# UWQuickstep/quickstep

Hardware: AMD Instinct MI355X
Metric: probe+aggregate rows/s at TPC-H SF100 (Q1,Q3) (higher is better)
Workload: dtype i32 keys / f64 sums

## Files before the change

### quickstep_amd/csrc/join.hip

```cpp

#include "common.hpp"
#include "join_dense.hpp"
#include "join_lds.hpp"
#include "scan.hpp"

#include <atomic>
#include <cstdlib>
#include <vector>
#include <mutex>
#include <shared_mutex>
#include <type_traits>

namespace qsx {

constexpr int kJBlock = 256;
constexpr uint64_t kEmpty64 = ~0ull;
constexpr uint32_t kEmptyTid = 0xFFFFFFFFu;

struct alignas(16) LongEntry {
  int64_t key;
  uint32_t tid;
  uint32_t pad;
};

// ... 559 lines not shown
      __syncthreads();
      const unsigned long long base = s_base;
      for (int i = threadIdx.x; i < staged; i += kJBlock) {
        const unsigned long long o = base + i;
        if (o < sink.capacity) {
          __builtin_nontemporal_store(s_probe[i], &out_probe[o]);
          __builtin_nontemporal_store(s_build[i], &out_build[o]);
        }
      }
      __syncthreads();
    }
  }
  if (MODE != 0) {
    local_count = wave_reduce_add(local_count);
    if (lane_id() == 0 && local_count != 0 && out_count != nullptr) atomicAdd(out_count, local_count);
  }
}

}
#include "join_lds_bucket.hpp"
namespace qsx {

struct KeyPackArgs {
  const void *cols[QSX_MAX_KEYS];
  int is_long[QSX_MAX_KEYS];
  int shift[QSX_MAX_KEYS];
  int ncols;
  int exact;
};

__device__ __forceinline__ uint64_t combine_hashes(uint64_t first, uint64_t second) {
  const uint64_t kMul = 0x9ddfea08eb382d69ull;
  uint64_t a = (first ^ second) * kMul;
  a ^= (a >> 47);
  uint64_t b = (second ^ a) * kMul;
  b ^= (b >> 47);
  b *= kMul;
  return b;
}

__global__ __launch_bounds__(kJBlock) void key_pack_kernel(KeyPackArgs a, int64_t n, int64_t *__restrict__ out) {
  for (int64_t i = static_cast<int64_t>(blockIdx.x) * kJBlock + threadIdx.x; i < n;
       i += static_cast<int64_t>(gridDim.x) * kJBlock) {
    uint64_t acc = 0;
    for (int k = 0; k < a.ncols; ++k) {
      const uint64_t v = a.is_long[k] ? static_cast<uint64_t>(static_cast<const int64_t *>(a.cols[k])[i])
                                      : static_cast<uint64_t>(static_cast<const uint32_t *>(a.cols[k])[i]);
      if (a.exact) acc |= v << a.shift[k];
      else acc = k == 0 ? v : combine_hashes(acc, v);
    }
    out[i] = static_cast<int64_t>(acc);
  }
}

__global__ __launch_bounds__(kJBlock) void key_pack_char_kernel(const unsigned char *__restrict__ col, int width, int64_t n,
                                                               int64_t *__restrict__ out) {
  for (int64_t i = static_cast<int64_t>(blockIdx.x) * kJBlock + threadIdx.x; i < n; i += static_cast<int64_t>(gridDim.x) * kJBlock) {
    uint64_t key = 0;
    bool ended = false;
    for (int b = 0; b < width; ++b) {
      const unsigned char c = col[i * width + b];
      ended = ended || c == 0;
      key |= static_cast<uint64_t>(ended ? 0 : c) << (8 * b);
    }
    out[i] = static_cast<int64_t>(key);
  }
}

__global__ __launch_bounds__(kJBlock) void key_pack_runs_kernel(KeyPackArgs a, const long long *__restrict__ runs, long long cols_offset,
                                                               int64_t *__restrict__ out, int coded) {
  constexpr int kTileRows = 512;
  const int lane = lane_id();
  const int num_tiles = static_cast<int>(runs[2]);
  for (int tile = __builtin_amdgcn_readfirstlane(static_cast<int>(blockIdx.x * (kJBlock / kWave) + (threadIdx.x >> 6))); tile < num_tiles;
       tile += static_cast<int>(gridDim.x) * (kJBlock / kWave)) {
    const RunTile at = run_locate(runs, tile);
    const long long n = run_rows(runs, at.block);
    const long long out_first = run_base(runs, at.block);
    const long long *cols = runs + cols_offset + static_cast<long long>(at.block) * a.ncols;
    const long long total_entries = runs[0] * a.ncols;
    const long long *widths = cols + total_entries, *dicts = widths + total_entries;
    for (int r = lane; r < kTileRows; r += kWave) {
      const long long i = static_cast<long long>(at.tile_in_block) * kTileRows + r;
      if (i >= n) break;
      uint64_t acc = 0;
      for (int k = 0; k < a.ncols; ++k) {
        const void *col = as_global(reinterpret_cast<const void *>(cols[k]));
        const int code_width = coded != 0 ? static_cast<int>(widths[k]) : 0;
        uint64_t v;
        if (code_width == 0) {
          v = a.is_long[k] ? static_cast<uint64_t>(static_cast<const int64_t *>(col)[i]) : static_cast<uint64_t>(static_cast<const uint32_t *>(col)[i]);
        } else {
          const uint32_t code = code_width == 1 ? static_cast<const uint8_t *>(col)[i]
                                                : (code_width == 2 ? static_cast<const uint16_t *>(col)[i] : static_cast<const uint32_t *>(col)[i]);
          const void *dict = as_global(reinterpret_cast<const void *>(dicts[k]));
          if (dict == nullptr) v = code;
          else v = a.is_long[k] ? static_cast<uint64_t>(static_cast<const int64_t *>(dict)[code]) : static_cast<uint64_t>(static_cast<const uint32_t *>(dict)[code]);
        }
        if (a.exact) acc |= v << a.shift[k];
        else acc = k == 0 ? v : combine_hashes(acc, v);
      }
      out[out_first + i] = static_cast<int64_t>(acc);
    }
  }
}

}

using namespace qsx;

struct qsx_join_table {
  int key_type = QSX_INT;
  uint64_t capacity = 0;
  void *slots = nullptr;
  unsigned long long *entries_dev = nullptr;
  int64_t reserved = 0;
  std::atomic<int64_t> max_tid{-1};
  std::shared_mutex mutex;


  std::mutex seal_mutex;
  std::atomic<int> seal_state{0};
  std::atomic<bool> scanned{false};
  std::mutex marks_mutex;
  std::vector<std::pair<hipStream_t, hipEvent_t>> marks;
  unsigned long long *control_host = nullptr;
  hipEvent_t seal_event = nullptr;
  hipStream_t seal_stream = nullptr;
  void *compact = nullptr;
  uint64_t compact_capacity = 0;
  CompactView compact_view() const {
    return CompactView{static_cast<const uint32_t *>(compact), static_cast<const unsigned char *>(compact) + compact_capacity * 4};
  }
  std::mutex cover_mutex;
  std::vector<long long> cover_sig;
  void *cover = nullptr;
  size_t cover_bytes = 0;
  int cover_entry_bytes = 0;
  int cover_state = 0;
  hipEvent_t cover_event = nullptr;
  hipStream_t cover_stream = nullptr;
  qsx_join_table *shadow = nullptr;

  bool dense = false;
  int64_t min_key = 0;
  int stride_shift = 0;
  uint64_t range = 0;
  uint32_t *head = nullptr;
  unsigned char *head3 = nullptr;
  hipEvent_t pack_event = nullptr;
  hipStream_t pack_stream = nullptr;
  uint2 *ov = nullptr;
  unsigned int ov_capacity = 0;
  DenseTableView dense_view() const {
    DenseTableView v;
    v.head = head;
    v.head3 = seal_state.load(std::memory_order_acquire) == 2 ? head3 : nullptr;
    v.ov = ov;
    v.min_key = min_key;
    v.stride_shift = stride_shift;
    v.range = range;
    v.ov_count = reinterpret_cast<unsigned int *>(entries_dev + 2);
    v.ov_capacity = ov_capacity;
    v.error = reinterpret_cast<int *>(entries_dev + 3);
    return v;
  }

  size_t entry_bytes() const { return key_type == QSX_INT ? 8 : 16; }
  size_t table_bytes() const { return capacity * entry_bytes() + capacity; }
  static size_t alloc_bytes(size_t entry, uint64_t cap) { return cap * entry + cap + cap / kBucketSlots * sizeof(unsigned int); }
  uint64_t room() const { return capacity / 5 * 4; }
  TableView view() const {
    TableView v{};
    v.slots = slots;
    v.dup_flag = reinterpret_cast<unsigned int *>(entries_dev + 2);
    v.fp = static_cast<unsigned char *>(slots) + capacity * entry_bytes();
    v.buckets = capacity / kBucketSlots;
    v.fill = reinterpret_cast<unsigned int *>(v.fp + capacity);
    return v;
  }
};
static void drop_cover(qsx_join_table *t);

constexpr size_t kControlBytes = static_cast<size_t>(kControlReplicas) * kControlStride * sizeof(unsigned long long);
static int reset_control_words(unsigned long long *control, hipStream_t stream) {
  QSX_HIP_TRY(hipMemsetAsync(control, 0, kControlBytes, stream));
  return QSX_OK;
}
static bool fold_control_words(const unsigned long long *copies, unsigned long long *v) {
  unsigned long long entries = 0, lo_inv = 0, hi = 0;
  for (int r = 0; r < kControlReplicas; ++r) {
    const unsigned long long *c = copies + static_cast<size_t>(r) * kControlStride;
    entries += c[0];
    lo_inv = c[4] > lo_inv ? c[4] : lo_inv;
    hi = c[5] > hi ? c[5] : hi;
  }
  v[0] = entries;
  v[1] = 0;
  v[2] = copies[2];
  v[3] = copies[3];
  v[4] = ~lo_inv;
  v[5] = hi;
  return !(lo_inv == 0 && hi == 0);
}
static int copy_control_words(const unsigned long long *control_dev, hipStream_t stream, unsigned long long *v, bool *any_key = nullptr) {
  unsigned long long copies[kControlReplicas * kControlStride];
  QSX_HIP_TRY(hipMemcpyAsync(copies, control_dev, kControlBytes, hipMemcpyDeviceToHost, stream));
  QSX_HIP_TRY(hipStreamSynchronize(stream));
  const bool any = fold_control_words(copies, v);
  if (any_key != nullptr) *any_key = any;
  return QSX_OK;
}

static void mark_stream(qsx_join_table *t, hipStream_t stream) {
  if (t->dense) return;
  std::lock_guard<std::mutex> lock(t->marks_mutex);
  for (auto &m : t->marks) {
    if (m.first == stream) {
      if (m.second != nullptr && hipEventRecord(m.second, stream) != hipSuccess) {
        (void)hipGetLastError();
        (void)hipEventDestroy(m.second);
        m.second = nullptr;
      }
      return;
    }
  }
  hipEvent_t e = nullptr;
  if (hipEventCreateWithFlags(&e, hipEventDisableTiming) != hipSuccess || hipEventRecord(e, stream) != hipSuccess) {
    (void)hipGetLastError();
    if (e != nullptr) (void)hipEventDestroy(e);
    e = nullptr;
  }
  t->marks.emplace_back(stream, e);
}

static uint64_t capacity_for(int key_type, int64_t entries) {
  (void)key_type;
  const uint64_t rows = static_cast<uint64_t>(entries < 512 ? 512 : entries);
  return (rows * 5 + 63) / 64 * kBucketSlots + kBucketSlots;
}

static int fill_empty(const qsx_join_table *t, void *slots, uint64_t capacity, hipStream_t stream) {
  QSX_HIP_TRY(hipMemsetAsync(slots, 0xFF, capacity * t->entry_bytes(), stream));
  QSX_HIP_TRY(hipMemsetAsync(static_cast<char *>(slots) + capacity * t->entry_bytes() + capacity, 0, capacity / kBucketSlots * sizeof(unsigned int), stream));
  return QSX_OK;
}

static int allocate_slots(qsx_join_table *t, uint64_t capacity, void **out) {
  QSX_HIP_TRY(device_malloc(out, qsx_join_table::alloc_bytes(t->entry_bytes(), capacity)));
  int rc = fill_empty(t, *out, capacity, nullptr);
  if (rc == QSX_OK) {
    const hipError_t waited = hipStreamSynchronize(nullptr);
    if (waited != hipSuccess) {
      set_last_error("hipStreamSynchronize(nullptr)", waited);
      rc = QSX_ERR_HIP;
    }
  }
  if (rc != QSX_OK) {
    (void)device_free(*out);
    *out = nullptr;
  }
  return rc;
}

static int ensure_room_dense(qsx_join_table *t, int64_t additional) {
  std::unique_lock<std::shared_mutex> lock(t->mutex);
  if (static_cast<uint64_t>(t->reserved + additional) <= t->ov_capacity) {
    t->reserved += additional;
    return QSX_OK;
  }
  QSX_HIP_TRY(hipDeviceSynchronize());
  uint64_t want = static_cast<uint64_t>(t->reserved + additional) * 2;
  if (want > 0x7FFFFFFFull) want = 0x7FFFFFFFull;
  if (want < static_cast<uint64_t>(t->reserved + additional)) return QSX_ERR_CAPACITY;
  uint2 *bigger = nullptr;
  QSX_HIP_TRY(device_malloc(reinterpret_cast<void **>(&bigger), want * sizeof(uint2)));
  if (t->ov_capacity != 0) {
    QSX_HIP_TRY(hipMemcpy(bigger, t->ov, static_cast<size_t>(t->ov_capacity) * sizeof(uint2), hipMemcpyDeviceToDevice));
  }
  (void)device_free(t->ov);
  t->ov = bigger;
  t->ov_capacity = static_cast<unsigned int>(want);
  t->reserved += additional;
  return QSX_OK;
}

static int ensure_room(qsx_join_table *t, int64_t additional) {
  if (t->dense) return ensure_room_dense(t, additional);
  std::unique_lock<std::shared_mutex> lock(t->mutex);
  if (static_cast<uint64_t>(t->reserved + additional) <= t->room()) {
    t->reserved += additional;
    return QSX_OK;
  }
  QSX_HIP_TRY(hipDeviceSynchronize());
  unsigned long long words[kControlWords];
  const int rc_words = copy_control_words(t->entries_dev, nullptr, words);
  if (rc_words != QSX_OK) return rc_words;
  const unsigned long long actual = words[0];
  t->reserved = static_cast<int64_t>(actual);
  if (static_cast<uint64_t>(t->reserved + additional) <= t->room()) {
    t->reserved += additional;
    return QSX_OK;
  }
  const uint64_t new_capacity = capacity_for(t->key_type, 2 * (t->reserved + additional));
  void *bigger = nullptr;
  int rc = allocate_slots(t, new_capacity, &bigger);
  if (rc != QSX_OK) return rc;
  TableView src = t->view();
  void *old_slots = t->slots;
  t->slots = bigger;
  t->capacity = new_capacity;
  TableView dst = t->view();
  hipLaunchKernelGGL(rehash_kernel, dim3(grid_for(static_cast<int64_t>(src.num_slots()), kJBlock)), dim3(kJBlock), 0, nullptr,
                     t->key_type == QSX_LONG ? 1 : 0, src, dst);
  QSX_CHECK_LAUNCH();
  QSX_HIP_TRY(hipDeviceSynchronize());
  QSX_HIP_TRY(device_free(old_slots));
  t->reserved += additional;
  return QSX_OK;
}

extern "C" {

int qsx_join_table_create(int key_type, int64_t est_entries, qsx_join_table_t **out) {
  QSX_REQUIRE_DEVICE();
  if (out == nullptr || est_entries < 0) return QSX_ERR_INVALID_ARGUMENT;
  if (key_type != QSX_INT && key_type != QSX_LONG) return QSX_ERR_UNSUPPORTED;
  qsx_join_table *t = new qsx_join_table();
  t->key_type = key_type;
  t->capacity = capacity_for(key_type, est_entries);
  int rc = allocate_slots(t, t->capacity, &t->slots);
  if (rc != QSX_OK) { delete t; return rc; }
  hipError_t err = device_malloc(reinterpret_cast<void **>(&t->entries_dev), kControlBytes);
  if (err == hipSuccess) err = hipMemset(t->entries_dev, 0, kControlBytes);
  if (err != hipSuccess) {
    set_last_error("device_malloc(entries)", err);
    (void)device_free(t->slots);
    delete t;
    return QSX_ERR_HIP;
  }
  *out = t;
  return QSX_OK;
}

int qsx_join_table_create_dense(int key_type, int64_t min_key, int64_t max_key, int64_t key_stride,
                                int64_t est_entries, qsx_join_table_t **out) {
  QSX_REQUIRE_DEVICE();
  if (out == nullptr || est_entries < 0 || max_key < min_key || key_stride < 1) return QSX_ERR_INVALID_ARGUMENT;
  if (key_type != QSX_INT && key_type != QSX_LONG) return QSX_ERR_UNSUPPORTED;
  if ((key_stride & (key_stride - 1)) != 0) return QSX_ERR_UNSUPPORTED;
  int stride_shift = 0;
  while ((1ll << stride_shift) < key_stride) ++stride_shift;
  const uint64_t span = static_cast<uint64_t>(max_key) - static_cast<uint64_t>(min_key);
  const uint64_t range = (span >> stride_shift) + 1;
  if (range > (1ull << 32)) return QSX_ERR_CAPACITY;
  qsx_join_table *t = new qsx_join_table();
  t->key_type = key_type;
  t->dense = true;
  t->min_key = min_key;
  t->stride_shift = stride_shift;
  t->range = range;
  t->ov_capacity = static_cast<unsigned int>(est_entries < 1024 ? 1024 : (est_entries > 0x7FFFFFFF ? 0x7FFFFFFF : est_entries));
  hipError_t err = device_malloc(reinterpret_cast<void **>(&t->head), range * sizeof(uint32_t));
  if (err == hipSuccess) err = hipMemset(t->head, 0, range * sizeof(uint32_t));
  if (err == hipSuccess) err = device_malloc(reinterpret_cast<void **>(&t->ov), static_cast<size_t>(t->ov_capacity) * sizeof(uint2));
  if (err == hipSuccess) err = device_malloc(reinterpret_cast<void **>(&t->entries_dev), kControlBytes);
  if (err == hipSuccess) err = hipMemset(t->entries_dev, 0, kControlBytes);
  if (err != hipSuccess) {
    set_last_error("device_malloc(dense join table)", err);
    (void)device_free(t->head);
    (void)device_free(t->ov);
    (void)device_free(t->entries_dev);
    delete t;
    return err == hipErrorOutOfMemory ? QSX_ERR_OUT_OF_MEMORY : QSX_ERR_HIP;
  }
  *out = t;
  return QSX_OK;
}

int qsx_join_key_pack(int ncols, const void *const *cols, const int32_t *types, int64_t n, int64_t *out_dev,
                      int *out_exact, qsx_stream_t stream) {
  QSX_REQUIRE_DEVICE();
  if (ncols < 1 || ncols > QSX_MAX_KEYS || cols == nullptr || types == nullptr || n < 0 || out_exact == nullptr ||
      (n > 0 && out_dev == nullptr)) {
    return QSX_ERR_INVALID_ARGUMENT;
  }
  KeyPackArgs a;
  a.ncols = ncols;
  int bits = 0;
  for (int k = 0; k < ncols; ++k) {
    if (types[k] != QSX_INT && types[k] != QSX_LONG) return QSX_ERR_UNSUPPORTED;
    if (n > 0 && cols[k] == nullptr) return QSX_ERR_INVALID_ARGUMENT;
    a.cols[k] = cols[k];
    a.is_long[k] = types[k] == QSX_LONG;
    a.shift[k] = bits < 64 ? bits : 0;
    bits += types[k] == QSX_LONG ? 64 : 32;
  }
  a.exact = bits <= 64;
  *out_exact = a.exact;
  if (n == 0) return QSX_OK;
  hipLaunchKernelGGL(key_pack_kernel, dim3(grid_for(n, kJBlock * 4)), dim3(kJBlock), 0, as_stream(stream), a, n, out_dev);
  QSX_CHECK_LAUNCH();
  return QSX_OK;
}

int qsx_join_key_pack_char(const void *col_dev, int width, int64_t n, int64_t *out_dev, qsx_stream_t stream) {
  QSX_REQUIRE_DEVICE();
  if (n < 0 || (n > 0 && (col_dev == nullptr || out_dev == nullptr))) return QSX_ERR_INVALID_ARGUMENT;
  if (width < 1 || width > 8) return QSX_ERR_UNSUPPORTED;
  if (n == 0) return QSX_OK;
  hipLaunchKernelGGL(key_pack_char_kernel, dim3(grid_for(n, kJBlock * 4)), dim3(kJBlock), 0, as_stream(stream),
                     static_cast<const unsigned char *>(col_dev), width, n, out_dev);
  QSX_CHECK_LAUNCH();
  return QSX_OK;
}

static int join_key_pack_blocks_impl(int ncols, const int32_t *types, int64_t num_blocks, const int64_t *block_rows,
                                     const void *const *block_cols, const int32_t *block_code_widths, const void *const *block_dictionaries,
                                     int64_t *out_dev, int *out_exact, qsx_stream_t stream) {
  QSX_REQUIRE_DEVICE();
  if (ncols < 1 || ncols > QSX_MAX_KEYS || types == nullptr || num_blocks < 0 || out_exact == nullptr ||
      (num_blocks > 0 && (block_rows == nullptr || block_cols == nullptr))) {
    return QSX_ERR_INVALID_ARGUMENT;
  }
  KeyPackArgs a;
  a.ncols = ncols;
  int bits = 0;
  for (int k = 0; k < ncols; ++k) {
    if (types[k] != QSX_INT && types[k] != QSX_LONG) return QSX_ERR_UNSUPPORTED;
    a.cols[k] = nullptr;
    a.is_long[k] = types[k] == QSX_LONG;
    a.shift[k] = bits < 64 ? bits : 0;
    bits += types[k] == QSX_LONG ? 64 : 32;
  }
  a.exact = bits <= 64;
  *out_exact = a.exact;
  std::vector<int64_t> first(static_cast<size_t>(num_blocks));
  std::vector<const void *> none(static_cast<size_t>(num_blocks), nullptr);
  int64_t total = 0;
  for (int64_t b = 0; b < num_blocks; ++b) {
    if (block_rows[b] < 0) return QSX_ERR_INVALID_ARGUMENT;
    first[b] = total;
    total += block_rows[b];
  }
  if (total == 0) return QSX_OK;
  if (out_dev == nullptr) return QSX_ERR_INVALID_ARGUMENT;
  std::vector<long long> table;
  const long long tiles = build_run_table(512, num_blocks, block_rows, none.data(), nullptr, nullptr, first.data(), &table);
  if (tiles < 0) return QSX_ERR_INVALID_ARGUMENT;
  const long long cols_offset = static_cast<long long>(table.size());
  for (int64_t b = 0; b < num_blocks; ++b) {
    for (int k = 0; k < ncols; ++k) {
      const void *col = block_cols[b * ncols + k];
      if (block_rows[b] > 0 && col == nullptr) return QSX_ERR_INVALID_ARGUMENT;
      table.push_back(static_cast<long long>(reinterpret_cast<uintptr_t>(col)));
    }
  }
  bool coded = false;
  for (int64_t e = 0; block_code_widths != nullptr && e < num_blocks * ncols; ++e) {
    const int w = block_code_widths[e];
    if (w != 0 && w != 1 && w != 2 && w != 4) return QSX_ERR_INVALID_ARGUMENT;
    coded = coded || w != 0;
  }
  if (coded) {
    for (int64_t e = 0; e < num_blocks * ncols; ++e) table.push_back(block_code_widths[e]);
    for (int64_t e = 0; e < num_blocks * ncols; ++e) {
      const void *d = block_dictionaries != nullptr && block_code_widths[e] != 0 ? block_dictionaries[e] : nullptr;
      table.push_back(static_cast<long long>(reinterpret_cast<uintptr_t>(d)));
    }
  }
  hipStream_t s = as_stream(stream);
  const size_t bytes = table.size() * sizeof(long long);
  const long long *runs_dev = static_cast<const long long *>(staged_device_buffer(s, bytes));
  if (runs_dev == nullptr) return QSX_ERR_OUT_OF_MEMORY;
  const int rc = staged_upload(s, table.data(), bytes);
  if (rc != QSX_OK) return rc;
  hipLaunchKernelGGL(key_pack_runs_kernel, dim3(grid_for(tiles, kJBlock / kWave)), dim3(kJBlock), 0, s, a, runs_dev, cols_offset, out_dev, coded ? 1 : 0);
  QSX_CHECK_LAUNCH();
  return QSX_OK;
}

int qsx_join_key_pack_blocks(int ncols, const int32_t *types, int64_t num_blocks, const int64_t *block_rows,
                             const void *const *block_cols, int64_t *out_dev, int *out_exact, qsx_stream_t stream) {
  return join_key_pack_blocks_impl(ncols, types, num_blocks, block_rows, block_cols, nullptr, nullptr, out_dev, out_exact, stream);
}
int qsx_join_key_pack_blocks_coded(int ncols, const int32_t *types, int64_t num_blocks, const int64_t *block_rows,
                                   const void *const *block_cols, const int32_t *block_code_widths, const void *const *block_dictionaries,
                                   int64_t *out_dev, int *out_exact, qsx_stream_t stream) {
  return join_key_pack_blocks_impl(ncols, types, num_blocks, block_rows, block_cols, block_code_widths, block_dictionaries, out_dev, out_exact, stream);
}

static int destroy_table(qsx_join_table_t *t, bool wait_for_device) {
  if (t == nullptr) return QSX_OK;
  if (wait_for_device) {
    (void)synchronize_owner_device(t->slots != nullptr ? static_cast<const void *>(t->slots) : static_cast<const void *>(t->head));
  }
  if (t->shadow != nullptr) (void)destroy_table(t->shadow, wait_for_device);
  (void)device_free_idle(t->slots);
  (void)device_free_idle(t->head);
  (void)device_free_idle(t->head3);
  (void)device_free_idle(t->compact);
  (void)device_free_idle(t->cover);
  if (t->pack_event != nullptr) (void)hipEventDestroy(t->pack_event);
  if (t->seal_event != nullptr) (void)hipEventDestroy(t->seal_event);
  for (auto &m : t->marks) {
    if (m.second != nullptr) (void)hipEventDestroy(m.second);
  }
  if (t->control_host != nullptr) (void)hipHostFree(t->control_host);
  (void)device_free_idle(t->ov);
  (void)device_free_idle(t->entries_dev);
  delete t;
  return QSX_OK;
}
int qsx_join_table_destroy(qsx_join_table_t *t) { return destroy_table(t, true); }
int qsx_join_table_release(qsx_join_table_t *t) { return destroy_table(t, false); }

int qsx_join_table_clear(qsx_join_table_t *t, qsx_stream_t stream) {
  QSX_REQUIRE_DEVICE();
  if (t == nullptr) return QSX_ERR_INVALID_ARGUMENT;
  std::unique_lock<std::shared_mutex> lock(t->mutex);
  if (t->dense) {
    QSX_HIP_TRY(hipMemsetAsync(t->head, 0, t->range * sizeof(uint32_t), as_stream(stream)));
  } else {
    const int rc_fill = fill_empty(t, t->slots, t->capacity, as_stream(stream));
    if (rc_fill != QSX_OK) return rc_fill;
  }
  const int rc_control = reset_control_words(t->entries_dev, as_stream(stream));
  if (rc_control != QSX_OK) return rc_control;
  t->reserved = 0;
  t->max_tid.store(-1);
  t->seal_state.store(0);
  t->scanned.store(false);
  drop_cover(t);
  mark_stream(t, as_stream(stream));
  return QSX_OK;
}

int qsx_join_table_size(qsx_join_table_t *t, int64_t *out_entries, qsx_stream_t stream) {
  QSX_REQUIRE_DEVICE();
  if (t == nullptr || out_entries == nullptr) return QSX_ERR_INVALID_ARGUMENT;
  unsigned long long v[kControlWords] = {0, 0, 0, 0, 0, 0};
  const int rc_words = copy_control_words(t->entries_dev, as_stream(stream), v);
  if (rc_words != QSX_OK) return rc_words;
  *out_entries = static_cast<int64_t>(v[0]);
  if (t->dense && static_cast<int>(v[3] & 0xFFFFFFFFu) != 0) return QSX_ERR_INVALID_ARGUMENT;
  return QSX_OK;
}

int qsx_join_build(qsx_join_table_t *t, const void *keys_dev, int64_t n, int32_t base_tid,
                   const uint64_t *filter_dev, qsx_stream_t stream) {
  QSX_REQUIRE_DEVICE();
  if (t == nullptr || n < 0 || base_tid < 0) return QSX_ERR_INVALID_ARGUMENT;
  if (n == 0) return QSX_OK;
  if (keys_dev == nullptr) return QSX_ERR_INVALID_ARGUMENT;
  if (static_cast<int64_t>(base_tid) + n > INT32_MAX) return QSX_ERR_INVALID_ARGUMENT;
  int rc = ensure_room(t, n);
  if (rc != QSX_OK) return rc;
  t->seal_state.store(0);
  t->scanned.store(false);
  drop_cover(t);
  for (int64_t seen = t->max_tid.load(); seen < base_tid + n - 1 && !t->max_tid.compare_exchange_weak(seen, base_tid + n - 1);) {}
  std::shared_lock<std::shared_mutex> lock(t->mutex);
  const int grid = grid_for(n, kJBlock * 4);
  if (t->dense) {
    const int dgrid = grid_for((n + 63) >> 6, (kDBlock / kWave) * kBuildR);
    if (t->key_type == QSX_INT) {
      hipLaunchKernelGGL(dense_build_kernel<int32_t>, dim3(dgrid), dim3(kDBlock), 0, as_stream(stream), t->dense_view(),
                         static_cast<const int32_t *>(keys_dev), n, base_tid, filter_dev, t->entries_dev);
    } else {
      hipLaunchKernelGGL(dense_build_kernel<int64_t>, dim3(dgrid), dim3(kDBlock), 0, as_stream(stream), t->dense_view(),
                         static_cast<const int64_t *>(keys_dev), n, base_tid, filter_dev, t->entries_dev);
    }
    QSX_CHECK_LAUNCH();
    return QSX_OK;
  }
  if (t->key_type == QSX_INT) {
    hipLaunchKernelGGL(build_kernel<int32_t>, dim3(grid), dim3(kJBlock), 0, as_stream(stream), t->view(),
                       static_cast<const int32_t *>(keys_dev), n, base_tid, filter_dev, t->entries_dev);
  } else {
    hipLaunchKernelGGL(build_kernel<int64_t>, dim3(grid), dim3(kJBlock), 0, as_stream(stream), t->view(),
                       static_cast<const int64_t *>(keys_dev), n, base_tid, filter_dev, t->entries_dev);
  }
  QSX_CHECK_LAUNCH();
  mark_stream(t, as_stream(stream));
  return QSX_OK;
}

static int check_key_coding(const qsx_key_coding_t **coding, int64_t num_blocks) {
  if (*coding == nullptr) return QSX_OK;
  if ((*coding)->block_code_width == nullptr) {
    *coding = nullptr;
    return QSX_OK;
  }
  bool any = false;
  for (int64_t b = 0; b < num_blocks; ++b) {
    const int w = (*coding)->block_code_width[b];
    if (w != 0 && w != 1 && w != 2 && w != 4) return QSX_ERR_INVALID_ARGUMENT;
    if (w == 0 && (*coding)->block_dictionaries != nullptr && (*coding)->block_dictionaries[b] != nullptr) return QSX_ERR_INVALID_ARGUMENT;
    any = any || w != 0;
  }
  if (!any) *coding = nullptr;
  return QSX_OK;
}

static int join_build_blocks_impl(qsx_join_table_t *t, int64_t num_blocks, const int64_t *block_rows, const void *const *block_keys,
                          const int32_t *block_base_tids, const uint64_t *const *block_filters, const qsx_key_coding_t *coding, qsx_stream_t stream) {
  QSX_REQUIRE_DEVICE();
  if (t == nullptr || num_blocks < 0 || (num_blocks > 0 && (block_rows == nullptr || block_keys == nullptr || block_base_tids == nullptr))) {
    return QSX_ERR_INVALID_ARGUMENT;
  }
  if (check_key_coding(&coding, num_blocks) != QSX_OK) return QSX_ERR_INVALID_ARGUMENT;
  std::vector<int64_t> base(static_cast<size_t>(num_blocks));
  int64_t total = 0;
  for (int64_t b = 0; b < num_blocks; ++b) {
    if (block_rows[b] < 0 || (block_rows[b] > 0 && block_keys[b] == nullptr) || block_base_tids[b] < 0 ||
        static_cast<int64_t>(block_base_tids[b]) + block_rows[b] > INT32_MAX) {
      return QSX_ERR_INVALID_ARGUMENT;
    }
    base[b] = block_base_tids[b];
    total += block_rows[b];
  }
  if (total == 0) return QSX_OK;
  int rc = ensure_room(t, total);
  if (rc != QSX_OK) return rc;
  t->seal_state.store(0);
  t->scanned.store(false);
  drop_cover(t);
  for (int64_t b = 0; b < num_blocks; ++b) {
    const int64_t last = base[b] + block_rows[b] - 1;
    for (int64_t seen = t->max_tid.load(); seen < last && !t->max_tid.compare_exchange_weak(seen, last);) {}
  }
  hipStream_t s = as_stream(stream);
  std::vector<long long> table;
  const long long groups = build_run_table(kBuildTile, num_blocks, block_rows, block_keys,
                                           reinterpret_cast<const void *const *>(block_filters), nullptr, base.data(), &table,
                                           coding != nullptr ? coding->block_code_width : nullptr,
                                           coding != nullptr ? coding->block_dictionaries : nullptr);
  if (groups < 0) return QSX_ERR_INVALID_ARGUMENT;
  const size_t bytes = table.size() * sizeof(long long);
  const long long *runs_dev = static_cast<const long long *>(staged_device_buffer(s, bytes));
  if (runs_dev == nullptr) return QSX_ERR_OUT_OF_MEMORY;
  rc = staged_upload(s, table.data(), bytes);
  if (rc != QSX_OK) return rc;
  std::shared_lock<std::shared_mutex> lock(t->mutex);
  if (t->dense) {
    const int dgrid = grid_for(groups, kDBlock / kWave);
    if (t->key_type == QSX_INT) {
      hipLaunchKernelGGL((dense_build_kernel<int32_t, true>), dim3(dgrid), dim3(kDBlock), 0, s, t->dense_view(),
                         static_cast<const int32_t *>(nullptr), total, 0, static_cast<const uint64_t *>(nullptr), t->entries_dev, runs_dev);
    } else {
      hipLaunchKernelGGL((dense_build_kernel<int64_t, true>), dim3(dgrid), dim3(kDBlock), 0, s, t->dense_view(),
                         static_cast<const int64_t *>(nullptr), total, 0, static_cast<const uint64_t *>(nullptr), t->entries_dev, runs_dev);
    }
  } else {
    const int grid = grid_for(groups, kJBlock / kWave);
    if (t->key_type == QSX_INT) {
      hipLaunchKernelGGL(build_runs_kernel<int32_t>, dim3(grid), dim3(kJBlock), 0, s, t->view(), runs_dev, t->entries_dev);
    } else {
      hipLaunchKernelGGL(build_runs_kernel<int64_t>, dim3(grid), dim3(kJBlock), 0, s, t->view(), runs_dev, t->entries_dev);
    }
  }
  QSX_CHECK_LAUNCH();
  mark_stream(t, s);
  return QSX_OK;
}

int qsx_join_build_blocks(qsx_join_table_t *t, int64_t num_blocks, const int64_t *block_rows, const void *const *block_keys,
                          const int32_t *block_base_tids, const uint64_t *const *block_filters, qsx_stream_t stream) {
  return join_build_blocks_impl(t, num_blocks, block_rows, block_keys, block_base_tids, block_filters, nullptr, stream);
}
int qsx_join_build_blocks_coded(qsx_join_table_t *t, int64_t num_blocks, const int64_t *block_rows, const void *const *block_keys,
                                const qsx_key_coding_t *coding, const int32_t *block_base_tids, const uint64_t *const *block_filters,
                                qsx_stream_t stream) {
  return join_build_blocks_impl(t, num_blocks, block_rows, block_keys, block_base_tids, block_filters, coding, stream);
}

}

static std::atomic<long long> g_compact_probes{0};
extern "C" long long qsx_debug_join_compact_probes(void) { return g_compact_probes.load(std::memory_order_relaxed); }
static bool lds_tables_enabled() {
  const char *e = getenv("QSX_JOIN_LDS");
  return e == nullptr || e[0] != '0';
}

static bool dense_two_pass(const uint64_t *filter) {
  const char *e = getenv("QSX_JOIN_TWO_PASS");
  if (e != nullptr && e[0] != '\0') return e[0] != '0';
  return filter != nullptr;
}

static void drop_cover(qsx_join_table *t) {
  std::lock_guard<std::mutex> lock(t->cover_mutex);
  t->cover_state = 0;
  t->cover_sig.clear();
}

constexpr int64_t kAdaptiveMinRows = 1 << 16;
static bool adaptive_enabled() {
  const char *e = getenv("QSX_JOIN_ADAPTIVE");
  return e == nullptr || e[0] != '0';
}

static void sealed_pack(qsx_join_table *t, hipStream_t stream) {
  auto behind_the_pack = [&]() {
    if (t->pack_stream != stream && t->pack_event != nullptr && hipEventQuery(t->pack_event) != hipSuccess) {
      (void)hipGetLastError();
      (void)hipStreamWaitEvent(stream, t->pack_event, 0);
    }
  };
  int state = t->seal_state.load(std::memory_order_acquire);
  if (state == 2) {
    behind_the_pack();
    return;
  }
  if (state != 0 || !adaptive_enabled()) return;
  const uint64_t bytes4 = t->range * 4, bytes3 = t->range * 3;
  if (bytes4 <= (13ull << 18) || bytes3 > (36ull << 20) / 10 || t->max_tid.load() >= (1 << 23) - 2 || t->reserved >= (1 << 23) - 1) {
    return;
  }
  std::lock_guard<std::mutex> lock(t->seal_mutex);
  state = t->seal_state.load(std::memory_order_acquire);
  if (state != 0) {
    if (state == 2) behind_the_pack();
    return;
  }
  if (t->head3 == nullptr && device_malloc(&t->head3, static_cast<size_t>(bytes3) + 4) != hipSuccess) {
    (void)hipGetLastError();
    t->head3 = nullptr;
    t->seal_state.store(1, std::memory_order_release);
    return;
  }
  if (t->pack_event == nullptr && hipEventCreateWithFlags(&t->pack_event, hipEventDisableTiming) != hipSuccess) {
    (void)hipGetLastError();
    t->pack_event = nullptr;
    t->seal_state.store(1, std::memory_order_release);
    return;
  }
  hipLaunchKernelGGL(dense_pack_kernel, dim3(grid_for(static_cast<int64_t>(t->range), kJBlock * 4)), dim3(kJBlock), 0, stream, t->head, t->range,
                     t->head3);
  if (hipGetLastError() != hipSuccess || hipEventRecord(t->pack_event, stream) != hipSuccess) {
    (void)hipGetLastError();
    (void)hipStreamSynchronize(stream);
    t->seal_state.store(1, std::memory_order_release);
    return;
  }
  t->pack_stream = stream;
  t->seal_state.store(2, std::memory_order_release);
}

static bool compact_enabled() {
  const char *e = getenv("QSX_JOIN_COMPACT");
  return e == nullptr || e[0] != '0';
}
static bool compact_possible(const qsx_join_table *t) {
  const uint64_t buckets = t->capacity / kBucketSlots;
  return compact_enabled() && t->key_type == QSX_INT && buckets >= kCompactMinBuckets && buckets <= 0xFFFFFFFFull && t->max_tid.load() < (1 << 24);
}
static bool seal_compact(qsx_join_table *t, bool duplicate_keys, hipStream_t stream) {
  if (!compact_possible(t) || duplicate_keys) return false;
  if (t->compact_capacity != t->capacity) {
    (void)device_free(t->compact);
    t->compact = nullptr;
    t->compact_capacity = 0;
    if (device_malloc(&t->compact, static_cast<size_t>(t->capacity) * 5 + 16) != hipSuccess) {
      (void)hipGetLastError();
      t->compact = nullptr;
      return false;
    }
    t->compact_capacity = t->capacity;
  }
  hipLaunchKernelGGL(compact_build_kernel, dim3(static_cast<unsigned>((t->capacity + kJBlock - 1) / kJBlock)), dim3(kJBlock), 0, stream, t->view(),
                     static_cast<uint32_t *>(t->compact), static_cast<unsigned char *>(t->compact) + t->capacity * 4);
  if (hipGetLastError() != hipSuccess) return false;
  return true;
}

static bool seal_verify_enabled() {
  const char *e = getenv("QSX_JOIN_SEAL_VERIFY");
  return e != nullptr && e[0] == '1';
}
static bool wait_for_builds(qsx_join_table *t, hipStream_t stream) {
  bool marked = true;
  std::lock_guard<std::mutex> lock(t->marks_mutex);
  for (const auto &m : t->marks) {
    if (m.second == nullptr) marked = false;
    else if (m.first != stream && hipStreamWaitEvent(stream, m.second, 0) != hipSuccess) marked = false;
  }
  if (!marked) (void)hipGetLastError();
  return marked;
}
static bool read_control_words(qsx_join_table *t, hipStream_t stream, unsigned long long *v, bool *any_key) {
  if (t->control_host == nullptr && hipHostMalloc(reinterpret_cast<void **>(&t->control_host), kControlBytes, hipHostMallocDefault) != hipSuccess) {
    (void)hipGetLastError();
    t->control_host = nullptr;
  }
  if (t->control_host == nullptr) return copy_control_words(t->entries_dev, stream, v, any_key) == QSX_OK;
  if (hipMemcpyAsync(t->control_host, t->entries_dev, kControlBytes, hipMemcpyDeviceToHost, stream) != hipSuccess ||
      hipStreamSynchronize(stream) != hipSuccess) {
    return false;
  }
  *any_key = fold_control_words(t->control_host, v);
  return true;
}
static void behind_the_seal(qsx_join_table *t, hipStream_t stream) {
  if (t->seal_stream != stream && t->seal_event != nullptr && hipEventQuery(t->seal_event) != hipSuccess) {
// ... 801 lines not shown
```

### quickstep_amd/csrc/join_dense.hpp

```cpp
#ifndef QSX_CSRC_JOIN_DENSE_HPP_
#define QSX_CSRC_JOIN_DENSE_HPP_

#include <type_traits>

#include "block_runs.hpp"
#include "common.hpp"

namespace qsx {

constexpr int kDBlock = 256;
constexpr int kDenseRowsPerThread = 16;
constexpr int kDenseTile = kDBlock * kDenseRowsPerThread;
constexpr uint32_t kChainBit = 0x80000000u;
constexpr int kDenseSparsePairs = 256;

struct DenseTableView {
  uint32_t *head;
  const unsigned char *head3;
  uint2 *ov;
  int64_t min_key;
  int stride_shift;
  uint64_t range;
  unsigned int *ov_count;
  unsigned int ov_capacity;
  int *error;
};

template <typename KeyT>
__device__ __forceinline__ uint64_t dense_index(const DenseTableView &t, KeyT key) {
  const uint64_t d = static_cast<uint64_t>(static_cast<int64_t>(key) - t.min_key);
  const uint64_t idx = d >> t.stride_shift;
  return (idx << t.stride_shift) == d && idx < t.range ? idx : ~0ull;
}

__device__ __forceinline__ uint32_t dense_head_word(const DenseTableView &t, uint64_t idx) {
  if (t.head3 == nullptr) return t.head[idx];
  uint32_t w;
  __builtin_memcpy(&w, t.head3 + idx * 3, 4);
  return (w & 0x7FFFFFu) | ((w & 0x800000u) << 8);
}

__device__ __forceinline__ bool dense_row_in_filter(const uint64_t *filter, int64_t row) {
  return filter == nullptr || ((filter[row >> 6] >> (63 - (row & 63))) & 1u);
}

constexpr int kBuildR = 8;
constexpr int kBuildTile = kBuildR * kWave;
template <typename KeyT, bool kRuns = false>
__global__ __launch_bounds__(kDBlock) void dense_build_kernel(DenseTableView t, const KeyT *__restrict__ keys, int64_t n,
                                                             int32_t base_tid_arg, const uint64_t *__restrict__ filter,
                                                             unsigned long long *__restrict__ entries,
                                                             const long long *__restrict__ runs = nullptr) {
  constexpr int R = kBuildR;
  using Source = ProbeTileSource<KeyT>;
  const int lane = lane_id();
  const int64_t num_groups = kRuns ? runs[2] : (((n + 63) >> 6) + R - 1) / R;
  const int64_t wave = __builtin_amdgcn_readfirstlane(static_cast<int>(blockIdx.x * (kDBlock / kWave) + (threadIdx.x >> 6)));
  const int64_t num_waves = static_cast<int64_t>(gridDim.x) * (kDBlock / kWave);
  unsigned long long inserted = 0;
  KeyT key[R], next_key[R];
  uint64_t words = ~0ull, next_words = ~0ull;
  auto source_of = [&](int64_t group) {
    return probe_tile_source<KeyT, kBuildTile, kRuns>(runs, group, keys, n, base_tid_arg, filter, nullptr);
  };
  auto request = [&](const Source &src, KeyT (&k)[R], uint64_t &fw) {
    const int64_t sw0 = src.base >> 6;
    if (kRuns && src.code_width != 0) {
      coded_keys(src, k, [&](int r) {
        const int64_t row = ((sw0 + r) << 6) + lane;
        return row < src.n ? row : src.n - 1;
      });
    } else {
#pragma unroll
      for (int r = 0; r < R; ++r) {
        const int64_t row = ((sw0 + r) << 6) + lane;
        k[r] = load_global(&src.keys[row < src.n ? row : src.n - 1]);
      }
    }
    fw = ~0ull;
    if (src.filter != nullptr && lane < R && sw0 + lane < ((src.n + 63) >> 6)) fw = load_global(&src.filter[sw0 + lane]);
  };
  Source cur = Source(), next = Source();
  int64_t group = wave;
  if (group < num_groups) {
    cur = source_of(group);
    request(cur, key, words);
  }
  for (; group < num_groups; group += num_waves) {
    if (group + num_waves < num_groups) {
      next = source_of(group + num_waves);
      request(next, next_key, next_words);
    }
    const int64_t w0 = cur.base >> 6;
    const int64_t n = cur.n;
    const int32_t base_tid = cur.base_tid;
    cur = next;
    uint64_t idx[R];
    uint32_t old[R];
#pragma unroll
    for (int r = 0; r < R; ++r) {
      const int64_t i = ((w0 + r) << 6) + lane;
      const uint64_t fw = __shfl(words, r, kWave);
      const bool live = i < n && msb_bit(fw, lane);
      idx[r] = live ? dense_index(t, key[r]) : ~1ull;
      if (idx[r] == ~0ull) atomicExch(t.error, 1);
      old[r] = 0u;
      if (idx[r] < ~1ull) old[r] = atomicCAS(&t.head[idx[r]], 0u, static_cast<uint32_t>(base_tid + i) + 1u);
    }
#pragma unroll
    for (int r = 0; r < R; ++r) {
      if (idx[r] >= ~1ull) continue;
      const int64_t i = ((w0 + r) << 6) + lane;
      const uint32_t tid = static_cast<uint32_t>(base_tid + i);
      if (old[r] != 0u) {
        const unsigned int e = atomicAdd(t.ov_count, 1u);
        if (e >= t.ov_capacity) {
          atomicExch(t.error, 2);
          continue;
        }
        t.ov[e].x = tid;
        t.ov[e].y = atomicExch(&t.head[idx[r]], kChainBit | e);
      }
      ++inserted;
    }
#pragma unroll
    for (int r = 0; r < R; ++r) key[r] = next_key[r];
    words = next_words;
  }
  inserted = wave_reduce_add(inserted);
  if (lane == 0 && inserted != 0) atomicAdd(entries + static_cast<size_t>(wave & 31) * 16, inserted);
}

constexpr int kProjColumnWords = 5;
struct ProjectionView {
  const long long *table;
  int nc;
  int nseg;
  int seg_rows;
  const void *cover;
  __device__ __forceinline__ int width(int c) const { return static_cast<int>(table[c]); }
  __device__ __forceinline__ bool on_build(int c) const { return table[nc + c] != 0; }
  __device__ __forceinline__ char *out(int c) const { return as_global(reinterpret_cast<char *>(table[2 * nc + c])); }
  __device__ __forceinline__ int cover_offset(int c) const { return static_cast<int>(table[3 * nc + c]); }
  __device__ __forceinline__ bool is_probe_key(int c) const { return table[4 * nc + c] != 0; }
  __device__ __forceinline__ const long long *first_tids() const { return table + kProjColumnWords * nc; }
  __device__ __forceinline__ const char *build_stripe(int seg, int c) const {
    return as_global(reinterpret_cast<const char *>(table[kProjColumnWords * nc + nseg + seg * nc + c]));
  }
  __device__ __forceinline__ const char *probe_stripe(int block, int c) const {
    return as_global(reinterpret_cast<const char *>(table[kProjColumnWords * nc + nseg + nseg * nc + block * nc + c]));
  }
};
__device__ __forceinline__ unsigned long long load_value(const char *src, int width) {
  switch (width) {
    case 1: return load_global(reinterpret_cast<const uint8_t *>(src));
    case 2: return load_global(reinterpret_cast<const uint16_t *>(src));
    case 4: return load_global(reinterpret_cast<const uint32_t *>(src));
    default: return load_global(reinterpret_cast<const unsigned long long *>(src));
  }
}
__device__ __forceinline__ void store_value(char *dst, unsigned long long v, int width) {
  switch (width) {
    case 1: store_global(static_cast<uint8_t>(v), reinterpret_cast<uint8_t *>(dst)); break;
    case 2: store_global(static_cast<uint16_t>(v), reinterpret_cast<uint16_t *>(dst)); break;
    case 4: store_global_nt(static_cast<uint32_t>(v), reinterpret_cast<uint32_t *>(dst)); break;
    default: store_global_nt(v, reinterpret_cast<unsigned long long *>(dst)); break;
  }
}
__device__ __forceinline__ const char *projected_build_value(const ProjectionView &p, int c, int width, uint32_t tid) {
  const long long *first = p.first_tids();
  int seg = 0;
  if (p.nseg > 1) {
    if (p.seg_rows > 0) {
      seg = static_cast<int>((tid - static_cast<uint32_t>(first[0])) / static_cast<uint32_t>(p.seg_rows));
      seg = seg < p.nseg ? seg : p.nseg - 1;
    } else {
      int lo = 0, hi = p.nseg - 1;
      while (lo < hi) {
        const int mid = (lo + hi + 1) >> 1;
        if (first[mid] <= static_cast<long long>(tid)) lo = mid; else hi = mid - 1;
      }
      seg = lo;
    }
  }
  return p.build_stripe(seg, c) + static_cast<size_t>(tid - static_cast<uint32_t>(first[seg])) * width;
}
template <typename KeyT>
__device__ __forceinline__ void project_one(const ProjectionView &p, const ProbeTileSource<KeyT> &tile, int64_t probe_row, uint32_t tid,
                                            unsigned long long o) {
  for (int c = 0; c < p.nc; ++c) {
    const int width = p.width(c);
    if (!p.on_build(c) && tile.code_width != 0 && p.is_probe_key(c)) {
      store_value(p.out(c) + o * width, static_cast<unsigned long long>(coded_key(tile, probe_row)), width);
      continue;
    }
    const char *src = p.on_build(c) ? projected_build_value(p, c, width, tid) : p.probe_stripe(tile.block, c) + static_cast<size_t>(probe_row) * width;
    store_value(p.out(c) + o * width, load_value(src, width), width);
  }
}

template <typename EntryT>
__global__ __launch_bounds__(kDBlock) void cover_build_kernel(DenseTableView t, ProjectionView p, EntryT *__restrict__ cover,
                                                             unsigned int *__restrict__ flags) {
  const uint64_t i = static_cast<uint64_t>(blockIdx.x) * kDBlock + threadIdx.x;
  if (i >= t.range) return;
  const uint32_t hw = t.head[i];
  unsigned long long words[2] = {~0ull, ~0ull};
  if (hw & kChainBit) {
    atomicOr(flags, 1u);
  } else if (hw != 0u) {
    words[0] = words[1] = 0ull;
    for (int c = 0; c < p.nc; ++c) {
      if (!p.on_build(c)) continue;
      const int width = p.width(c), off = p.cover_offset(c);
      const unsigned long long v = load_value(projected_build_value(p, c, width, hw - 1u), width);
      if (off < 8) words[0] |= v << (8 * off); else words[1] |= v << (8 * (off - 8));
    }
    const bool ones = sizeof(EntryT) == 4 ? static_cast<uint32_t>(words[0]) == ~0u
                                          : (sizeof(EntryT) == 8 ? words[0] == ~0ull : (words[0] & words[1]) == ~0ull);
    if (ones) atomicOr(flags, 2u);
  }
  if constexpr (sizeof(EntryT) == 4) {
    cover[i] = static_cast<uint32_t>(words[0]);
  } else if constexpr (sizeof(EntryT) == 8) {
    cover[i] = words[0];
  } else {
    cover[i] = EntryT{words[0], words[1]};
  }
}

__device__ __forceinline__ void dense_emit_direct(bool match, int32_t probe_tid, int32_t build_tid,
                                                  int32_t *__restrict__ out_probe, int32_t *__restrict__ out_build,
                                                  unsigned long long capacity, unsigned long long *out_count) {
  const uint64_t m = __ballot(match);
  if (m == 0) return;
  unsigned long long base = 0;
  if (lane_id() == __ffsll(static_cast<long long>(m)) - 1) {
    base = atomicAdd(out_count, static_cast<unsigned long long>(__popcll(m)));
  }
  base = __shfl(base, __ffsll(static_cast<long long>(m)) - 1, kWave);
  const unsigned long long o = base + rank_below(m);
  if (match && o < capacity) {
    __builtin_nontemporal_store(probe_tid, &out_probe[o]);
    __builtin_nontemporal_store(build_tid, &out_build[o]);
  }
}

template <typename KeyT, int MODE, bool kRuns = false>
__global__ __launch_bounds__(kDBlock) __attribute__((amdgpu_waves_per_eu(MODE == 5 ? 3 : 1))) void dense_probe_kernel(
    DenseTableView t, const KeyT *__restrict__ keys, int64_t n, int32_t probe_base_tid,
    const uint64_t *__restrict__ filter, int32_t *__restrict__ out_probe, int32_t *__restrict__ out_build,
    int64_t capacity_signed, unsigned long long *__restrict__ out_count, uint64_t *__restrict__ out_bitmap, int anti,
    int32_t *__restrict__ unit_counts = nullptr, const int64_t *__restrict__ unit_offsets = nullptr,
    const long long *__restrict__ runs = nullptr, ProjectionView proj = ProjectionView{}) {
  constexpr int R = kDenseRowsPerThread;
  constexpr bool kProject = MODE == 5;
  using Source = ProbeTileSource<KeyT>;
  const unsigned long long capacity = static_cast<unsigned long long>(capacity_signed);
  const int64_t num_tiles = kRuns ? runs[2] : (n + kDenseTile - 1) / kDenseTile;
  auto source_of = [&](int64_t tile) {
    return probe_tile_source<KeyT, kDenseTile, kRuns>(runs, tile, keys, n, probe_base_tid, filter, out_bitmap);
  };
  unsigned long long local_count = 0;
  __shared__ int2 s_sparse[(MODE == 0 || MODE == 4) ? kDBlock / kWave : 1][(MODE == 0 || MODE == 4) ? kDenseSparsePairs : 1];
  __shared__ int s_wave_total[2][kDBlock / kWave];
  __shared__ unsigned long long s_tile_base;
  int parity = 0;
  const int wave = threadIdx.x >> 6;

  const int lane = lane_id();
  KeyT key[R], next_key[R];
  uint64_t filter_words = ~0ull, next_filter_words = ~0ull;
  auto request = [&](const Source &src, KeyT (&k)[R], uint64_t &words) {
    if (kRuns && src.code_width != 0) {
      coded_keys(src, k, [&](int r) {
        const int64_t row = src.base + r * kDBlock + threadIdx.x;
        return row < src.n ? row : src.n - 1;
      });
    } else {
#pragma unroll
      for (int r = 0; r < R; ++r) {
        const int64_t row = src.base + r * kDBlock + threadIdx.x;
        k[r] = load_global_nt(&src.keys[row < src.n ? row : src.n - 1]);
// ... 381 lines not shown
```

Before: 180.7 billion.

## Replace atomic CAS dense build with plain-store, verify and link passes on first build

On the first build into a cleared dense join table, the CAS-based insert is replaced by three passes. Pass one writes head words with plain stores, pass two reads them back and appends the losing rows to the overflow array using wave-aggregated atomics, and a link kernel then chains the overflow entries. Later builds wait on an event and fall back to the CAS kernel. The aim is to remove per-row atomic CAS contention and per-row overflow atomics, at the cost of an extra pass over the keys and two extra launches.

New measurement: 181.4 billion (median of 5 runs). No clear change (+0.4%).

```diff
diff --git a/quickstep_amd/csrc/join.hip b/quickstep_amd/csrc/join.hip
--- a/quickstep_amd/csrc/join.hip
+++ b/quickstep_amd/csrc/join.hip
@@ -735,6 +735,10 @@
   hipStream_t pack_stream = nullptr;
   uint2 *ov = nullptr;
   unsigned int ov_capacity = 0;
+  std::mutex build_mutex;
+  bool first_build = true;
+  bool build_event_live = false;
+  hipEvent_t build_event = nullptr;
   DenseTableView dense_view() const {
     DenseTableView v;
     v.head = head;
@@ -900,6 +904,52 @@
   QSX_HIP_TRY(hipDeviceSynchronize());
   QSX_HIP_TRY(device_free(old_slots));
   t->reserved += additional;
+  return QSX_OK;
+}
+
+static std::atomic<long long> g_exclusive_builds{0};
+extern "C" long long qsx_debug_join_exclusive_builds(void) { return g_exclusive_builds.load(std::memory_order_relaxed); }
+static bool exclusive_build_enabled() {
+  const char *e = getenv("QSX_JOIN_EXCLUSIVE_BUILD");
+  return e == nullptr || e[0] != '0';
+}
+constexpr int kLinkGrid = 64;
+
+template <typename KeyT, bool kRuns>
+static void launch_dense_build(int pass, int grid, hipStream_t s, const DenseTableView &v, const KeyT *keys, int64_t n, int32_t base_tid,
+                               const uint64_t *filter, unsigned long long *entries, const long long *runs) {
+  auto kernel = pass == 0 ? &dense_build_kernel<KeyT, kRuns, 0> : (pass == 1 ? &dense_build_kernel<KeyT, kRuns, 1> : &dense_build_kernel<KeyT, kRuns, 2>);
+  hipLaunchKernelGGL(kernel, dim3(grid), dim3(kDBlock), 0, s, v, keys, n, base_tid, filter, entries, runs);
+}
+
+template <typename Launch>
+static int dense_build(qsx_join_table *t, hipStream_t s, Launch launch) {
+  {
+    std::lock_guard<std::mutex> lock(t->build_mutex);
+    const bool first = t->first_build;
+    t->first_build = false;
+    if (first && exclusive_build_enabled()) {
+      if (t->build_event == nullptr && hipEventCreateWithFlags(&t->build_event, hipEventDisableTiming) != hipSuccess) {
+        (void)hipGetLastError();
+        t->build_event = nullptr;
+      }
+      if (t->build_event != nullptr) {
+        launch(1);
+        QSX_CHECK_LAUNCH();
+        launch(2);
+        QSX_CHECK_LAUNCH();
+        hipLaunchKernelGGL(dense_link_kernel, dim3(kLinkGrid), dim3(kDBlock), 0, s, t->dense_view());
+        QSX_CHECK_LAUNCH();
+        QSX_HIP_TRY(hipEventRecord(t->build_event, s));
+        t->build_event_live = true;
+        g_exclusive_builds.fetch_add(1, std::memory_order_relaxed);
+        return QSX_OK;
+      }
+    }
+    if (t->build_event_live) QSX_HIP_TRY(hipStreamWaitEvent(s, t->build_event, 0));
+  }
+  launch(0);
+  QSX_CHECK_LAUNCH();
   return QSX_OK;
 }
 
@@ -1085,6 +1135,7 @@
   (void)device_free_idle(t->compact);
   (void)device_free_idle(t->cover);
   if (t->pack_event != nullptr) (void)hipEventDestroy(t->pack_event);
+  if (t->build_event != nullptr) (void)hipEventDestroy(t->build_event);
   if (t->seal_event != nullptr) (void)hipEventDestroy(t->seal_event);
   for (auto &m : t->marks) {
     if (m.second != nullptr) (void)hipEventDestroy(m.second);
@@ -1104,6 +1155,9 @@
   std::unique_lock<std::shared_mutex> lock(t->mutex);
   if (t->dense) {
     QSX_HIP_TRY(hipMemsetAsync(t->head, 0, t->range * sizeof(uint32_t), as_stream(stream)));
+    std::lock_guard<std::mutex> build_lock(t->build_mutex);
+    t->first_build = true;
+    t->build_event_live = false;
   } else {
     const int rc_fill = fill_empty(t, t->slots, t->capacity, as_stream(stream));
     if (rc_fill != QSX_OK) return rc_fill;
@@ -1147,15 +1201,16 @@
   const int grid = grid_for(n, kJBlock * 4);
   if (t->dense) {
     const int dgrid = grid_for((n + 63) >> 6, (kDBlock / kWave) * kBuildR);
-    if (t->key_type == QSX_INT) {
-      hipLaunchKernelGGL(dense_build_kernel<int32_t>, dim3(dgrid), dim3(kDBlock), 0, as_stream(stream), t->dense_view(),
-                         static_cast<const int32_t *>(keys_dev), n, base_tid, filter_dev, t->entries_dev);
-    } else {
-      hipLaunchKernelGGL(dense_build_kernel<int64_t>, dim3(dgrid), dim3(kDBlock), 0, as_stream(stream), t->dense_view(),
-                         static_cast<const int64_t *>(keys_dev), n, base_tid, filter_dev, t->entries_dev);
-    }
-    QSX_CHECK_LAUNCH();
-    return QSX_OK;
+    hipStream_t s = as_stream(stream);
+    return dense_build(t, s, [&](int pass) {
+      if (t->key_type == QSX_INT) {
+        launch_dense_build<int32_t, false>(pass, dgrid, s, t->dense_view(), static_cast<const int32_t *>(keys_dev), n, base_tid, filter_dev,
+                                           t->entries_dev, nullptr);
+      } else {
+        launch_dense_build<int64_t, false>(pass, dgrid, s, t->dense_view(), static_cast<const int64_t *>(keys_dev), n, base_tid, filter_dev,
+                                           t->entries_dev, nullptr);
+      }
+    });
   }
   if (t->key_type == QSX_INT) {
     hipLaunchKernelGGL(build_kernel<int32_t>, dim3(grid), dim3(kJBlock), 0, as_stream(stream), t->view(),
@@ -1228,13 +1283,13 @@
   std::shared_lock<std::shared_mutex> lock(t->mutex);
   if (t->dense) {
     const int dgrid = grid_for(groups, kDBlock / kWave);
-    if (t->key_type == QSX_INT) {
-      hipLaunchKernelGGL((dense_build_kernel<int32_t, true>), dim3(dgrid), dim3(kDBlock), 0, s, t->dense_view(),
-                         static_cast<const int32_t *>(nullptr), total, 0, static_cast<const uint64_t *>(nullptr), t->entries_dev, runs_dev);
-    } else {
-      hipLaunchKernelGGL((dense_build_kernel<int64_t, true>), dim3(dgrid), dim3(kDBlock), 0, s, t->dense_view(),
-                         static_cast<const int64_t *>(nullptr), total, 0, static_cast<const uint64_t *>(nullptr), t->entries_dev, runs_dev);
-    }
+    return dense_build(t, s, [&](int pass) {
+      if (t->key_type == QSX_INT) {
+        launch_dense_build<int32_t, true>(pass, dgrid, s, t->dense_view(), nullptr, total, 0, nullptr, t->entries_dev, runs_dev);
+      } else {
+        launch_dense_build<int64_t, true>(pass, dgrid, s, t->dense_view(), nullptr, total, 0, nullptr, t->entries_dev, runs_dev);
+      }
+    });
   } else {
     const int grid = grid_for(groups, kJBlock / kWave);
     if (t->key_type == QSX_INT) {
diff --git a/quickstep_amd/csrc/join_dense.hpp b/quickstep_amd/csrc/join_dense.hpp
--- a/quickstep_amd/csrc/join_dense.hpp
+++ b/quickstep_amd/csrc/join_dense.hpp
@@ -46,7 +46,7 @@
 
 constexpr int kBuildR = 8;
 constexpr int kBuildTile = kBuildR * kWave;
-template <typename KeyT, bool kRuns = false>
+template <typename KeyT, bool kRuns = false, int PASS = 0>
 __global__ __launch_bounds__(kDBlock) void dense_build_kernel(DenseTableView t, const KeyT *__restrict__ keys, int64_t n,
                                                              int32_t base_tid_arg, const uint64_t *__restrict__ filter,
                                                              unsigned long long *__restrict__ entries,
@@ -103,12 +103,40 @@
       const uint64_t fw = __shfl(words, r, kWave);
       const bool live = i < n && msb_bit(fw, lane);
       idx[r] = live ? dense_index(t, key[r]) : ~1ull;
-      if (idx[r] == ~0ull) atomicExch(t.error, 1);
+      if (PASS != 2 && idx[r] == ~0ull) atomicExch(t.error, 1);
       old[r] = 0u;
-      if (idx[r] < ~1ull) old[r] = atomicCAS(&t.head[idx[r]], 0u, static_cast<uint32_t>(base_tid + i) + 1u);
+      if (idx[r] < ~1ull) {
+        const uint32_t word = static_cast<uint32_t>(base_tid + i) + 1u;
+        if constexpr (PASS == 0) old[r] = atomicCAS(&t.head[idx[r]], 0u, word);
+        else if constexpr (PASS == 1) t.head[idx[r]] = word;
+        else old[r] = t.head[idx[r]];
+      }
+    }
+    if constexpr (PASS == 1) {
+#pragma unroll
+      for (int r = 0; r < R; ++r) inserted += idx[r] < ~1ull ? 1u : 0u;
+    } else if constexpr (PASS == 2) {
+#pragma unroll
+      for (int r = 0; r < R; ++r) {
+        const uint32_t tid = static_cast<uint32_t>(base_tid + ((w0 + r) << 6) + lane);
+        const bool lost = idx[r] < ~1ull && old[r] != tid + 1u;
+        const uint64_t lm = __ballot(lost);
+        if (lm == 0) continue;
+        const int leader = __ffsll(static_cast<long long>(lm)) - 1;
+        unsigned int e0 = 0;
+        if (lane == leader) e0 = atomicAdd(t.ov_count, static_cast<unsigned int>(__popcll(lm)));
+        const unsigned int e = __shfl(e0, leader, kWave) + rank_below(lm);
+        if (!lost) continue;
+        if (e >= t.ov_capacity) {
+          atomicExch(t.error, 2);
+          continue;
+        }
+        t.ov[e] = make_uint2(tid, static_cast<uint32_t>(idx[r]));
+      }
     }
 #pragma unroll
     for (int r = 0; r < R; ++r) {
+      if (PASS != 0) break;
       if (idx[r] >= ~1ull) continue;
       const int64_t i = ((w0 + r) << 6) + lane;
       const uint32_t tid = static_cast<uint32_t>(base_tid + i);
@@ -129,6 +157,15 @@
   }
   inserted = wave_reduce_add(inserted);
   if (lane == 0 && inserted != 0) atomicAdd(entries + static_cast<size_t>(wave & 31) * 16, inserted);
+}
+
+__global__ __launch_bounds__(kDBlock) void dense_link_kernel(DenseTableView t) {
+  const unsigned int appended = *t.ov_count;
+  const unsigned int count = appended < t.ov_capacity ? appended : t.ov_capacity;
+  for (unsigned int e = blockIdx.x * kDBlock + threadIdx.x; e < count; e += gridDim.x * kDBlock) {
+    const uint32_t idx = t.ov[e].y;
+    t.ov[e].y = atomicExch(&t.head[idx], kChainBit | e);
+  }
 }
 
 constexpr int kProjColumnWords = 5;
```
